# irfanfadhullah/unet_zoo

Hardware: AMD Instinct MI355X
Metric: images/sec (fwd+bwd) at B=16 3x256x256, 1/2/4/8 MI355X (higher is better)
Workload: dtype bf16; 1 GPU; unet train step (zero_grad+fwd+BCE+bwd+clip+AdamW), B=16/GPU 3x256x256, random-init weights; global_batch=16, parallelism=dp1

## Files before the change

unet_zoo_amd/csrc/uz_common.h:

```cpp
#pragma once
#include <hip/hip_runtime.h>
#include <stdarg.h>
#include <stdint.h>
#include <stdio.h>
#include "../../include/unetzoo_hip.h"

typedef __bf16 bf16_t;
typedef __attribute__((ext_vector_type(16))) float f32x16;
typedef __attribute__((ext_vector_type(4))) float f32x4;
typedef __attribute__((ext_vector_type(8))) __bf16 bf16x8;
typedef __attribute__((ext_vector_type(4))) __bf16 bf16x4;

#include <hip/hip_ext.h>
bool uz_prof_take(hipEvent_t* e0, hipEvent_t* e1);
#undef hipLaunchKernelGGL
#define hipLaunchKernelGGL(kern, grid, block, shm, stream, ...)                                              \
  do {                                                                                                       \
    hipEvent_t uz_e0_, uz_e1_;                                                                               \
    if (uz_prof_take(&uz_e0_, &uz_e1_))                                                                      \
      hipExtLaunchKernelGGL(kern, dim3(grid), dim3(block), (shm), (stream), uz_e0_, uz_e1_, 0, __VA_ARGS__);   \
    else                                                                                                     \
      kern<<<dim3(grid), dim3(block), (shm), (stream)>>>(__VA_ARGS__);                                       \
  } while (0)

// ... 109 lines not shown
  const char* e = getenv("UZ_TUNE");
  return e ? atoi(e) : 0;
}
static inline const char* uz_ablate_env(const char* name) { return getenv(name); }
#else
static inline int uz_tune_flags() { return 0; }
static inline const char* uz_ablate_env(const char*) { return nullptr; }
#endif

struct UzDirectPlan {
  int tw, bn, bres, th_n, tw_n, ntiles, tiles_n, grid_m;
  int ppcfg;
  int ksplit, cps;
};
int uz_direct_plan(const uz_conv_desc* d, UzDirectPlan* p);
struct UzBnRed {
  const void* y;
  int ldy;
  const float *scale, *shift, *mean, *invstd;
};
struct UzXf {
  const float *scale, *shift;
};
struct UzBnAct {
  const float *scale, *shift;
  int relu;
};
int uz_direct_launch(const uz_conv_desc* d, const UzDirectPlan& p, const void* x, const void* w,
                     const float* bias, void* y, float* stats, hipStream_t s, const UzBnRed* br = nullptr,
                     float* part = nullptr,
                     const UzXf* xf = nullptr, const UzBnAct* ba = nullptr);

enum { UZ_PP_512 = 0,
       UZ_PP_512X64 = 1,
       UZ_PP_256 = 2,
       UZ_PP_256W16 = 3,
       UZ_PP_128W16 = 4 };
struct UzPpPlan {
  int cfg, bn, th_n, tw_n, ntiles, tiles_n, grid_m;
  int ksplit, cps;
};
int uz_pp_plan(const uz_conv_desc* d, UzPpPlan* p);
int uz_pp_launch(const uz_conv_desc* d, const UzPpPlan& p, const void* x, const void* w, const float* bias, void* y,
                 float* stats, hipStream_t s, const UzBnRed* br = nullptr, float* part = nullptr, const UzXf* xf = nullptr,
                 const UzBnAct* ba = nullptr);
int uz_pp_xf_channels(const UzPpPlan& p);

struct UzWgrad2Plan {
  int big, one_tap, gather, kw, kr, tiles_i, tiles_j, kg, units, upb, split, nslabs, H, W;
  int wide9;
  int v9, bi;
};
int uz_wgrad9_plan(const uz_wgrad_desc* d, UzWgrad2Plan* p);
int uz_wgrad9_launch(const uz_wgrad_desc* d, const UzWgrad2Plan& p, const void* L, const void* R, float* slab, hipStream_t s,
                     const UzXf* xf = nullptr);
const char* uz_wgrad9_name(const UzWgrad2Plan& p);
int uz_wgrad_g4_plan(const uz_wgrad_desc* d, UzWgrad2Plan* p);
int uz_wgrad_g4_launch(const uz_wgrad_desc* d, const UzWgrad2Plan& p, const void* L, const void* R, float* slab, hipStream_t s);
int uz_wgrad3x3_plan(const uz_wgrad_desc* d, UzWgrad2Plan* p, int batch = 1);
int uz_wgrad3x3_launch(const uz_wgrad_desc* d, const UzWgrad2Plan& p, const void* L, const void* R,
                       float* slab, hipStream_t s, int batch = 1, long long lb_bytes = 0, long long rb_bytes = 0,
                       long long slab_stride = 0,
                       int batch2 = 1, long long lb2_bytes = 0, long long rb2_bytes = 0,
                       const UzXf* xf = nullptr);

struct UzWgradMultiItem {
  const uz_wgrad_desc* d;
  UzWgrad2Plan p;
  const void *L, *R;
  float* slab;
};
int uz_wgrad3x3_multi_max();
int uz_wgrad3x3_multi_launch(const UzWgradMultiItem* items, int n, hipStream_t s);

struct UzGemmPlan {
  int bn, bm, nst, tiles_m, tiles_n, grid_m;
  int ksplit, cps;
};
int uz_gemm_dma_plan(const uz_conv_desc* d, UzGemmPlan* p);
long long uz_gemm_dma_workspace_bytes(const uz_conv_desc* d);
int uz_gemm_dma_launch(const uz_conv_desc* d, const UzGemmPlan& p, const void* x, const void* w,
                       const float* bias, void* y, float* stats, hipStream_t s, const void* res = nullptr,
                       int ldres = 0, const UzBnRed* br = nullptr, float* part = nullptr);
```

unet_zoo_amd/csrc/uz_igemm.hip:

```cpp
#include "uz_common.h"
#include <string.h>

namespace {

struct IgemmArgs {
  const void* x;
  const void* w;
  void* y;
  const float* bias;
  float* stats;
  int M, H, W, Hin, Win, Cin, ldx, Nout, ldy, K, ntaps, mode, dil, store, Co, tiles_m, Hout, Wout;
  float* part;
  int tpg;
  const float* act_scale;
  const float* act_shift;
  int act_relu;
};

template <typename T> struct Mma;
template <> struct Mma<bf16_t> {
  static __device__ __forceinline__ void run(const Vec16<bf16_t>& a, const Vec16<bf16_t>& b,
                                             f32x16& c) {
    c = __builtin_amdgcn_mfma_f32_32x32x16_bf16(*reinterpret_cast<const bf16x8*>(&a),
                                                *reinterpret_cast<const bf16x8*>(&b), c, 0, 0, 0);
// ... 373 lines not shown
    UZ_REQUIRE(d->dil >= 1, "uz_conv_igemm: dil=%d", d->dil);
  } else if (d->taps_mode == UZ_TAPS_CONV_S2) {
    UzGemmPlan gs2_;
    UZ_REQUIRE(d->ntaps == 9 && d->store_mode == UZ_STORE_PLAIN && d->H == (d->Hin + 1) / 2 && d->W == (d->Win + 1) / 2,
               "uz_conv_igemm: stride-2 taps need ntaps=9, a plain store and H = ceil(Hin/2), W = ceil(Win/2)");
    UZ_REQUIRE(uz_gemm_dma_plan(d, &gs2_), "uz_conv_igemm: stride-2 taps need the LDS-DMA GEMM (channel multiples, tensor < 2 GiB)");
  } else {
    UZ_REQUIRE(d->taps_mode == UZ_TAPS_GATHER2X2 && d->ntaps == 4,
               "uz_conv_igemm: gather2x2 needs ntaps=4");
    UZ_REQUIRE((d->Hin == 2 * d->H || d->Hin == 2 * d->H + 1) && (d->Win == 2 * d->W || d->Win == 2 * d->W + 1),
               "uz_conv_igemm: gather2x2 needs Hin in {2H, 2H+1}, Win in {2W, 2W+1}");
  }
  if (d->store_mode == UZ_STORE_SHUFFLE2X2) {
    UZ_REQUIRE(d->Co > 0 && d->Nout == 4 * d->Co, "uz_conv_igemm: shuffle store needs Nout=4*Co");
    UZ_REQUIRE((d->Hout == 0 || d->Hout == 2 * d->H || d->Hout == 2 * d->H + 1) &&
                   (d->Wout == 0 || d->Wout == 2 * d->W || d->Wout == 2 * d->W + 1),
               "uz_conv_igemm: shuffle store destination must be 2H..2H+1 x 2W..2W+1");
    UZ_REQUIRE(d->ldy >= d->Co, "uz_conv_igemm: bad ldy");
  } else {
    UZ_REQUIRE(d->store_mode == UZ_STORE_PLAIN, "uz_conv_igemm: bad store_mode");
    UZ_REQUIRE(d->ldy >= d->Nout, "uz_conv_igemm: bad ldy=%d (Nout=%d)", d->ldy, d->Nout);
  }
  const long long M = (long long)d->N * d->H * d->W;
  UZ_REQUIRE(M * (long long)(d->ldx > d->ldy ? d->ldx : d->ldy) < (1LL << 40) && M < (1LL << 31),
             "uz_conv_igemm: tensor too large");
  UZ_REQUIRE((long long)d->N * d->Hin * d->Win < (1LL << 31), "uz_conv_igemm: input too large");
  p->bn = d->Nout <= 64 ? 64 : 128;
  p->tiles_m = uz_cdiv(M, 128);
  p->tiles_n = uz_cdiv(d->Nout, p->bn);
  int cap = (2 * UZ_NUM_CU) / p->tiles_n;
  if (cap < 1) cap = 1;
  p->grid_m = p->tiles_m < cap ? p->tiles_m : cap;
  p->split = 1;
  const int vec_ = d->dtype == UZ_BF16 ? 8 : 4;
  if (d->taps_mode == UZ_TAPS_CONV && d->ntaps == 9 && d->store_mode == UZ_STORE_PLAIN &&
      p->tiles_m * p->tiles_n <= UZ_NUM_CU / 2 && d->Nout % vec_ == 0 && d->ldy % vec_ == 0 &&
      !(uz_tune_flags() & 8)) {
    p->split = 9;
    reduce_geometry(M, d->Nout, vec_, p);
  }
  return UZ_OK;
}

template <typename T>
int launch(const uz_conv_desc* d, const Plan& p, const IgemmArgs& a, hipStream_t s) {
  dim3 grid(p.grid_m, p.tiles_n, a.part != nullptr ? p.split : 1), block(256);
  if (a.act_scale != nullptr) {
    if (p.bn == 64) hipLaunchKernelGGL((igemm_kernel<T, 128, 64, 2, 2, true>), grid, block, 0, s, a);
    else hipLaunchKernelGGL((igemm_kernel<T, 128, 128, 2, 2, true>), grid, block, 0, s, a);
    UZ_LAUNCH_CHECK("uz_conv_igemm_bnact");
    return UZ_OK;
  }
  if (p.bn == 64) {
    hipLaunchKernelGGL((igemm_kernel<T, 128, 64, 2, 2>), grid, block, 0, s, a);
  } else {
    hipLaunchKernelGGL((igemm_kernel<T, 128, 128, 2, 2>), grid, block, 0, s, a);
  }
  UZ_LAUNCH_CHECK("uz_conv_igemm");
  if (a.part != nullptr) {
    constexpr int VEC = ElemTraits<T>::VEC;
    const size_t shm = (size_t)256 * 2 * VEC * sizeof(float);
    hipLaunchKernelGGL((igemm_split_reduce_kernel<T>), dim3(p.rgx, p.rgy), dim3(p.rbx, p.rby), shm, s,
                       static_cast<const float*>(a.part), p.split, a.M, a.Nout, a.bias, static_cast<T*>(a.y), a.ldy, a.stats,
                       static_cast<const T*>(nullptr), 0);
    UZ_LAUNCH_CHECK("uz_conv_igemm(split reduce)");
  }
  return UZ_OK;
}

bool generic_path(const uz_conv_desc* d) {
  UzDirectPlan dp;
  UzGemmPlan gp;
  return !uz_direct_plan(d, &dp) && !uz_gemm_dma_plan(d, &gp);
}

}

extern "C" int uz_conv_igemm_grid_m(const uz_conv_desc* d) {
  Plan p;
  const int rc = make_plan(d, &p);
  if (rc != UZ_OK) return rc;
  UzDirectPlan dp;
  if (uz_direct_plan(d, &dp)) return dp.grid_m;
  UzGemmPlan gp;
  if (uz_gemm_dma_plan(d, &gp)) return gp.grid_m;
  return p.grid_m;
}

extern "C" int uz_conv_igemm_kernel_name(const uz_conv_desc* d, int with_workspace, char* buf, int cap) {
  Plan p;
  const int rc = make_plan(d, &p);
  if (rc != UZ_OK) return rc;
  UZ_REQUIRE(buf != nullptr && cap > 0, "uz_conv_igemm_kernel_name: no buffer");
  const char* dt = d->dtype == UZ_BF16 ? "bf16" : "f32";
  char name[96];
  UzDirectPlan dp;
  UzGemmPlan gp;
  if (uz_direct_plan(d, &dp)) {
    const char* up = d->taps_mode == UZ_TAPS_CONV_UP2 ? "_up2" : "";
    static const char* const ppn[8] = {"pp512", "pp512x64", "pp256", "pp256w16", "pp128w16", "?", "?", "?"};
    if (dp.bres == 3) snprintf(name, sizeof(name), "conv3x3_%s_%s%s%s", ppn[dp.ppcfg & 7], dt, up, (dp.ksplit > 1 && with_workspace) ? "_splitk" : "");
    else if (dp.bres == 2) snprintf(name, sizeof(name), "conv3x3_res64_%s%s", dt, up);
    else snprintf(name, sizeof(name), "conv3x3_direct_%s_bn%d%s%s", dt, dp.bn, dp.bres == 1 ? "_resident" : "", up);
  } else if (uz_gemm_dma_plan(d, &gp)) {
    snprintf(name, sizeof(name), "gemm_dma_%s", dt);
  } else {
    snprintf(name, sizeof(name), "igemm_%s_128x%d%s", dt, p.bn, (p.split > 1 && with_workspace) ? "_tapsplit" : "");
  }
  const int len = (int)strlen(name);
  snprintf(buf, (size_t)cap, "%s", name);
  return len;
}

extern "C" long long uz_conv_igemm_workspace_bytes(const uz_conv_desc* d) {
  Plan p;
  const int rc = make_plan(d, &p);
  if (rc != UZ_OK) return rc;
  {
    UzDirectPlan dp;
    if (uz_direct_plan(d, &dp) && dp.bres == 3 && dp.ksplit > 1)
      return (long long)dp.ksplit * d->N * d->H * d->W * d->Nout * (long long)sizeof(float);
  }
  {
    UzDirectPlan dp;
    const long long gb = uz_direct_plan(d, &dp) ? 0 : uz_gemm_dma_workspace_bytes(d);
    if (gb > 0) return gb;
  }
  if (p.split <= 1 || !generic_path(d)) return 0;
  return (long long)p.split * d->N * d->H * d->W * d->Nout * (long long)sizeof(float);
}

extern "C" int uz_conv_igemm_ws_grid_m(const uz_conv_desc* d) {
  Plan p;
  const int rc = make_plan(d, &p);
  if (rc != UZ_OK) return rc;
  {
    UzDirectPlan dp;
    if (uz_direct_plan(d, &dp) && dp.bres == 3 && dp.ksplit > 1) {
      Plan rp;
      reduce_geometry((long long)d->N * d->H * d->W, d->Nout, 8, &rp);
      return rp.rgx;
    }
  }
  {
    UzDirectPlan dp;
    if (!uz_direct_plan(d, &dp) && uz_gemm_dma_workspace_bytes(d) > 0) {
      Plan rp;
      reduce_geometry((long long)d->N * d->H * d->W, d->Nout, 8, &rp);
      return rp.rgx;
    }
  }
  if (p.split > 1 && generic_path(d)) return p.rgx;
  return uz_conv_igemm_grid_m(d);
}

extern "C" int uz_conv_igemm(const uz_conv_desc* d, const void* x, const void* w_packed,
                             const float* bias, void* y, float* stats_partial, void* stream) {
  return uz_conv_igemm_ws(d, x, w_packed, bias, y, stats_partial, nullptr, stream);
}

static int gemm_split_k(const uz_conv_desc* d, const UzGemmPlan& gp, const void* x, const void* w_packed, const float* bias,
                        const void* res, int ldres, void* y, void* workspace, hipStream_t s, float* stats = nullptr) {
  const int r1 = uz_gemm_dma_launch(d, gp, x, w_packed, nullptr, y, nullptr, s, nullptr, 0, nullptr, static_cast<float*>(workspace));
  if (r1 != UZ_OK) return r1;
  Plan rp;
  const long long M = (long long)d->N * d->H * d->W;
  reduce_geometry(M, d->Nout, 8, &rp);
  const size_t shm = (size_t)256 * 2 * 8 * sizeof(float);
  hipLaunchKernelGGL((igemm_split_reduce_kernel<bf16_t>), dim3(rp.rgx, rp.rgy), dim3(rp.rbx, rp.rby), shm, s,
                     static_cast<const float*>(workspace), gp.ksplit, (int)M, d->Nout, bias, static_cast<bf16_t*>(y), d->ldy,
                     stats, static_cast<const bf16_t*>(res), ldres);
  UZ_LAUNCH_CHECK("uz_conv_igemm(split-K GEMM reduce)");
  return UZ_OK;
}

extern "C" int uz_conv_igemm_res(const uz_conv_desc* d, const void* x, const void* w_packed, const float* bias,
                                 const void* res, int ldres, void* y, void* stream) {
  return uz_conv_igemm_res_ws(d, x, w_packed, bias, res, ldres, y, nullptr, stream);
}

extern "C" int uz_conv_igemm_res_ws(const uz_conv_desc* d, const void* x, const void* w_packed, const float* bias,
                                    const void* res, int ldres, void* y, void* workspace, void* stream) {
  Plan p;
  const int rc = make_plan(d, &p);
  if (rc != UZ_OK) return rc;
  UZ_REQUIRE(x && w_packed && y && res, "uz_conv_igemm_res: null pointer");
  UZ_REQUIRE(((uintptr_t)x & 15) == 0 && ((uintptr_t)w_packed & 15) == 0 && ((uintptr_t)y & 15) == 0 &&
                 ((uintptr_t)res & 15) == 0, "uz_conv_igemm_res: x / w / y / res must be 16-byte aligned");
  const int vec = d->dtype == UZ_BF16 ? 8 : 4;
  UZ_REQUIRE(ldres >= d->Nout && ldres % vec == 0, "uz_conv_igemm_res: bad ldres %d", ldres);
  UzDirectPlan dp;
  UzGemmPlan gp;
  if (d->store_mode != UZ_STORE_PLAIN || uz_direct_plan(d, &dp) || !uz_gemm_dma_plan(d, &gp)) {
    uz_set_error("uz_conv_igemm_res: only problems of the LDS-DMA GEMM with a plain store take a residual");
    return UZ_ENOTIMPL;
  }
  if (gp.ksplit > 1 && workspace != nullptr)
    return gemm_split_k(d, gp, x, w_packed, bias, res, ldres, y, workspace, static_cast<hipStream_t>(stream));
  return uz_gemm_dma_launch(d, gp, x, w_packed, bias, y, nullptr, static_cast<hipStream_t>(stream), res, ldres);
}

extern "C" int uz_conv_igemm_xf_supported(const uz_conv_desc* d) {
  UzDirectPlan dp;
  if (d == nullptr || d->dtype != UZ_BF16) return 0;
  if (!uz_direct_plan(d, &dp) || dp.bres != 3 || dp.ksplit > 1) return 0;
  UzPpPlan pp = {dp.ppcfg, dp.bn, dp.th_n, dp.tw_n, dp.ntiles, dp.tiles_n, dp.grid_m, dp.ksplit, dp.cps};
  return d->Cin <= uz_pp_xf_channels(pp) ? 1 : 0;
}

extern "C" int uz_conv_igemm_xf(const uz_conv_desc* d, const void* x, const float* in_scale, const float* in_shift,
                                const void* w_packed, const float* bias, void* y, float* stats_partial, void* stream) {
  Plan p;
  const int rc = make_plan(d, &p);
  if (rc != UZ_OK) return rc;
  UZ_REQUIRE(x && w_packed && y && in_scale && in_shift, "uz_conv_igemm_xf: null pointer");
  UZ_REQUIRE(((uintptr_t)x & 15) == 0 && ((uintptr_t)w_packed & 15) == 0 && ((uintptr_t)y & 15) == 0,
             "uz_conv_igemm_xf: x / w / y must be 16-byte aligned");
  if (!uz_conv_igemm_xf_supported(d)) {
    uz_set_error("uz_conv_igemm_xf: only bf16 3x3 problems of the ping-pong configurations whose LDS image leaves room for "
                 "the channel table (ask uz_conv_igemm_xf_supported)");
    return UZ_ENOTIMPL;
  }
  UzDirectPlan dp;
  UZ_REQUIRE(uz_direct_plan(d, &dp), "uz_conv_igemm_xf: no plan");
  const UzXf xf = {in_scale, in_shift};
  return uz_direct_launch(d, dp, x, w_packed, bias, y, stats_partial, static_cast<hipStream_t>(stream), nullptr, nullptr, &xf);
}

extern "C" int uz_conv_igemm_bnred_supported(const uz_conv_desc* d) {
  UzDirectPlan dp;
  UzGemmPlan gp;
  if (d == nullptr || d->dtype != UZ_BF16) return 0;
  if (uz_direct_plan(d, &dp)) return dp.bres != 2 ? 1 : 0;
  return (d->store_mode == UZ_STORE_PLAIN && uz_gemm_dma_plan(d, &gp)) ? 1 : 0;
}

extern "C" int uz_conv_igemm_bnred(const uz_conv_desc* d, const void* x, const void* w_packed, void* y,
                                   const void* bn_y, int ld_bny, const float* scale, const float* shift,
                                   const float* mean, const float* invstd, float* partial, void* stream) {
  Plan p;
  const int rc = make_plan(d, &p);
  if (rc != UZ_OK) return rc;
  UZ_REQUIRE(x && w_packed && y && bn_y && scale && shift && mean && invstd && partial,
             "uz_conv_igemm_bnred: null pointer");
  UZ_REQUIRE(((uintptr_t)x & 15) == 0 && ((uintptr_t)w_packed & 15) == 0 && ((uintptr_t)y & 15) == 0 &&
                 ((uintptr_t)bn_y & 15) == 0, "uz_conv_igemm_bnred: x / w / y / bn_y must be 16-byte aligned");
  UZ_REQUIRE(ld_bny >= d->Nout && ld_bny % 8 == 0, "uz_conv_igemm_bnred: bad ld_bny %d", ld_bny);
  UzDirectPlan dp;
  UzGemmPlan gp;
  if (!uz_conv_igemm_bnred_supported(d)) {
    uz_set_error("uz_conv_igemm_bnred: only bf16 problems of the direct 3x3 kernels with the LDS-staged epilogue and of "
                 "the LDS-DMA GEMM with a plain store (ask uz_conv_igemm_bnred_supported)");
    return UZ_ENOTIMPL;
  }
  const UzBnRed br = {bn_y, ld_bny, scale, shift, mean, invstd};
  if (uz_direct_plan(d, &dp))
    return uz_direct_launch(d, dp, x, w_packed, nullptr, y, partial, static_cast<hipStream_t>(stream), &br);
  UZ_REQUIRE(uz_gemm_dma_plan(d, &gp), "uz_conv_igemm_bnred: no plan");
  return uz_gemm_dma_launch(d, gp, x, w_packed, nullptr, y, partial, static_cast<hipStream_t>(stream), nullptr, 0, &br);
}

extern "C" int uz_conv_igemm_ws(const uz_conv_desc* d, const void* x, const void* w_packed,
                                const float* bias, void* y, float* stats_partial, void* workspace,
                                void* stream) {
  Plan p;
  const int rc = make_plan(d, &p);
  if (rc != UZ_OK) return rc;
  UZ_REQUIRE(x && w_packed && y, "uz_conv_igemm: null pointer");
  UZ_REQUIRE(((uintptr_t)x & 15) == 0 && ((uintptr_t)w_packed & 15) == 0 && ((uintptr_t)y & 15) == 0,
             "uz_conv_igemm: x / w / y must be 16-byte aligned");
  UzDirectPlan dp;
  if (uz_direct_plan(d, &dp)) {
    if (dp.bres == 3 && dp.ksplit > 1 && workspace != nullptr) {
      hipStream_t s = static_cast<hipStream_t>(stream);
      const int r1 = uz_direct_launch(d, dp, x, w_packed, nullptr, y, nullptr, s, nullptr, static_cast<float*>(workspace));
      if (r1 != UZ_OK) return r1;
      Plan rp;
      const long long M = (long long)d->N * d->H * d->W;
      reduce_geometry(M, d->Nout, 8, &rp);
      const size_t shm = (size_t)256 * 2 * 8 * sizeof(float);
      hipLaunchKernelGGL((igemm_split_reduce_kernel<bf16_t>), dim3(rp.rgx, rp.rgy), dim3(rp.rbx, rp.rby), shm, s,
                         static_cast<const float*>(workspace), dp.ksplit, (int)M, d->Nout, bias, static_cast<bf16_t*>(y), d->ldy,
                         stats_partial, static_cast<const bf16_t*>(nullptr), 0);
      UZ_LAUNCH_CHECK("uz_conv_igemm(split-K reduce)");
      return UZ_OK;
    }
    return uz_direct_launch(d, dp, x, w_packed, bias, y, stats_partial, static_cast<hipStream_t>(stream));
  }
  UzGemmPlan gp;
  if (uz_gemm_dma_plan(d, &gp)) {
    if (gp.ksplit > 1 && workspace != nullptr)
      return gemm_split_k(d, gp, x, w_packed, bias, nullptr, 0, y, workspace, static_cast<hipStream_t>(stream), stats_partial);
    return uz_gemm_dma_launch(d, gp, x, w_packed, bias, y, stats_partial, static_cast<hipStream_t>(stream));
  }
  IgemmArgs a;
  a.x = x;
  a.w = w_packed;
  a.y = y;
  a.bias = bias;
  a.stats = stats_partial;
  a.M = d->N * d->H * d->W;
  a.H = d->H;
  a.W = d->W;
  a.Hin = d->Hin;
  a.Win = d->Win;
  a.Cin = d->Cin;
  a.ldx = d->ldx;
  a.Nout = d->Nout;
  a.ldy = d->ldy;
  a.K = d->ntaps * d->Cin;
  a.ntaps = d->ntaps;
  a.mode = d->taps_mode;
  a.dil = d->dil;
  a.store = d->store_mode;
  a.Co = d->Co;
  a.Hout = d->Hout ? d->Hout : 2 * d->H;
  a.Wout = d->Wout ? d->Wout : 2 * d->W;
  a.tiles_m = p.tiles_m;
  a.part = (p.split > 1 && workspace != nullptr) ? static_cast<float*>(workspace) : nullptr;
  a.tpg = (d->ntaps + p.split - 1) / p.split;
  a.act_scale = nullptr;
  a.act_shift = nullptr;
  a.act_relu = 0;
  hipStream_t s = static_cast<hipStream_t>(stream);
  return d->dtype == UZ_BF16 ? launch<bf16_t>(d, p, a, s) : launch<float>(d, p, a, s);
}

extern "C" int uz_conv_igemm_bnact_supported(const uz_conv_desc* d) {
  Plan p;
  if (d == nullptr || make_plan(d, &p) != UZ_OK) return 0;
  if (d->store_mode != UZ_STORE_PLAIN || !(d->taps_mode == UZ_TAPS_CONV || d->taps_mode == UZ_TAPS_CONV_UP2)) return 0;
  UzDirectPlan dp;
  UzGemmPlan gp;
  if (uz_direct_plan(d, &dp)) {
    if (dp.bres == 2) return 0;
    if (dp.bres == 3 && dp.ksplit > 1) return 0;
    return 1;
  }
  if (uz_gemm_dma_plan(d, &gp)) return 0;
  return p.split > 1 ? 0 : 1;
}

extern "C" int uz_conv_igemm_bnact(const uz_conv_desc* d, const void* x, const void* w_packed, const float* bias,
                                   const float* out_scale, const float* out_shift, int relu, void* y, void* stream) {
  Plan p;
  const int rc = make_plan(d, &p);
  if (rc != UZ_OK) return rc;
  UZ_REQUIRE(x && w_packed && y && out_scale && out_shift, "uz_conv_igemm_bnact: null pointer");
  UZ_REQUIRE(((uintptr_t)x & 15) == 0 && ((uintptr_t)w_packed & 15) == 0 && ((uintptr_t)y & 15) == 0 &&
                 ((uintptr_t)out_scale & 15) == 0 && ((uintptr_t)out_shift & 15) == 0,
             "uz_conv_igemm_bnact: x / w / y / out_scale / out_shift must be 16-byte aligned");
  if (!uz_conv_igemm_bnact_supported(d)) {
    uz_set_error("uz_conv_igemm_bnact: only plain-store 3x3 / 1x1 problems of the direct kernels with a workgroup-wide "
                 "epilogue and of the generic kernel, without a split plan (ask uz_conv_igemm_bnact_supported)");
    return UZ_ENOTIMPL;
  }
  hipStream_t s = static_cast<hipStream_t>(stream);
  const UzBnAct ba = {out_scale, out_shift, relu ? 1 : 0};
  UzDirectPlan dp;
  if (uz_direct_plan(d, &dp)) return uz_direct_launch(d, dp, x, w_packed, bias, y, nullptr, s, nullptr, nullptr, nullptr, &ba);
  IgemmArgs a;
  a.x = x;
  a.w = w_packed;
  a.y = y;
  a.bias = bias;
  a.stats = nullptr;
  a.M = d->N * d->H * d->W;
  a.H = d->H;
  a.W = d->W;
  a.Hin = d->Hin;
  a.Win = d->Win;
// ... 21 lines not shown
```

unet_zoo_amd/ops.py:

```python
from __future__ import annotations

import ctypes
import math
from ctypes import byref
from typing import List, Optional, Sequence

import torch

from . import _lib as L


class Act:

    __slots__ = ("buf", "off", "C", "N", "H", "W", "grads", "parts", "rparts", "needs_grad", "colsums", "bn_src",
                 "bn_partials", "lazy", "_taken")

    def __init__(self, buf: torch.Tensor, off: int, C: int, N: int, H: int, W: int, needs_grad: bool = True):
        assert buf.dim() == 2 and buf.is_contiguous() and buf.shape[0] == N * H * W
        assert 0 <= off and off + C <= buf.shape[1]
        self.buf, self.off, self.C, self.N, self.H, self.W = buf, off, C, N, H, W
        self.grads: List["Act"] = []
        self.parts: Optional[Sequence["Act"]] = None
        self.rparts: Optional[Sequence[tuple]] = None
        self.needs_grad = needs_grad
# ... 221 lines not shown

def conv_first_wgrad(x: torch.Tensor, dy: Act, out: Optional[torch.Tensor] = None) -> torch.Tensor:
    L.require_cuda(x, dy.buf)
    N, C, H, W = x.shape
    Cout = dy.C
    lib = L.load()
    ws_bytes = L.check_count(lib.uz_conv3x3_first_wgrad_workspace_bytes(N, H, W, Cout), "uz_conv3x3_first_wgrad_workspace_bytes")
    ws = torch.empty(ws_bytes // 4, dtype=torch.float32, device=x.device)
    if out is None:
        out = torch.empty((Cout, C, 3, 3), dtype=torch.float32, device=x.device)
    assert out.numel() == Cout * C * 9 and out.is_contiguous() and out.dtype == torch.float32
    with _Timed("wgrad_first_bf16", 2.0 * N * H * W * 9 * C * Cout, 4.0 * x.numel() + 2.0 * dy.P * Cout):
        L.check(lib.uz_conv3x3_first_wgrad(L.dtype_code(dy.dtype), x.data_ptr(), N, C, H, W, dy.ptr(), dy.ld, Cout,
                                           out.data_ptr(), ws.data_ptr(), L.stream_ptr()), "uz_conv3x3_first_wgrad")
    return out


def conv_first_wgrad_bn(x: torch.Tensor, g: Act, y: Act, vec: torch.Tensor, sums: torch.Tensor,
                        out: Optional[torch.Tensor] = None) -> torch.Tensor:
    L.require_cuda(x, g.buf, y.buf)
    N, C, H, W = x.shape
    Cout = g.C
    assert (y.N, y.H, y.W, y.C) == (g.N, g.H, g.W, g.C) == (N, H, W, Cout) and g.dtype == y.dtype == torch.bfloat16
    assert sums.dtype == torch.float64 and sums.shape == (2, Cout) and sums.is_contiguous()
    lib = L.load()
    ws_bytes = L.check_count(lib.uz_conv3x3_first_wgrad_workspace_bytes(N, H, W, Cout), "uz_conv3x3_first_wgrad_workspace_bytes")
    ws = torch.empty(ws_bytes // 4, dtype=torch.float32, device=x.device)
    if out is None:
        out = torch.empty((Cout, C, 3, 3), dtype=torch.float32, device=x.device)
    assert out.numel() == Cout * C * 9 and out.is_contiguous() and out.dtype == torch.float32
    with _Timed("wgrad_first_bf16", 2.0 * N * H * W * 9 * C * Cout, 4.0 * x.numel() + 4.0 * g.P * Cout):
        L.check(lib.uz_conv3x3_first_wgrad_bn(L.dtype_code(g.dtype), x.data_ptr(), N, C, H, W, g.ptr(), g.ld, y.ptr(), y.ld,
                                              vec[0].data_ptr(), vec[1].data_ptr(), vec[2].data_ptr(), vec[3].data_ptr(),
                                              sums.data_ptr(), float(y.P), Cout, out.data_ptr(), ws.data_ptr(), L.stream_ptr()),
                "uz_conv3x3_first_wgrad_bn")
    return out


def conv_kernel_name(d, with_workspace: bool = False) -> str:
    buf = ctypes.create_string_buffer(96)
    L.check_count(L.load().uz_conv_igemm_kernel_name(byref(d), 1 if with_workspace else 0, buf, 96),
                  "uz_conv_igemm_kernel_name")
    return buf.value.decode()


def _conv_desc(x: Act, nout: int, ldy: int, ntaps: int, taps_mode: int, dil: int = 1, store_mode: int = L.STORE_PLAIN,
               co: int = 0, Hd: int = 0, Wd: int = 0):
    if taps_mode == L.TAPS_CONV:
        H, W = x.H, x.W
    elif taps_mode == L.TAPS_CONV_UP2:
        H, W = 2 * x.H, 2 * x.W
    elif taps_mode == L.TAPS_CONV_S2:
        H, W = (x.H + 1) // 2, (x.W + 1) // 2
    else:
        H, W = x.H // 2, x.W // 2
    return L.ConvDesc(L.dtype_code(x.dtype), x.N, H, W, x.H, x.W, x.C, x.ld, nout, ldy, ntaps, taps_mode, dil, store_mode, co,
                      Hd, Wd)


def _wgrad_desc(Lt: Act, Rt: Act, ntaps: int, taps_mode: int = L.TAPS_CONV, dil: int = 1):
    return L.WgradDesc(L.dtype_code(Lt.dtype), Lt.N, Lt.H, Lt.W, Rt.H, Rt.W, Lt.C, Lt.ld, Rt.C, Rt.ld, ntaps, taps_mode, dil)


def conv_igemm(x: Act, w_packed: torch.Tensor, bias: Optional[torch.Tensor], y: Act, *,
               ntaps: int, dil: int = 1, taps_mode: int = L.TAPS_CONV,
               store_mode: int = L.STORE_PLAIN, nout: Optional[int] = None, co: int = 0,
               want_stats: bool = False, res: Optional[Act] = None,
               bnred: Optional[tuple] = None, xform: Optional[tuple] = None) -> Optional[torch.Tensor]:
    L.require_cuda(x.buf, w_packed, y.buf)
    lib = L.load()
    shuffle = store_mode == L.STORE_SHUFFLE2X2
    d = _conv_desc(x, nout if nout is not None else y.C, y.ld, ntaps, taps_mode, dil, store_mode, co,
                   y.H if shuffle else 0, y.W if shuffle else 0)
    assert w_packed.dtype == x.dtype and y.dtype == x.dtype
    assert w_packed.shape == (d.Nout, ntaps * x.C), (tuple(w_packed.shape), d.Nout, ntaps, x.C)
    stats = None
    if want_stats:
        gm = L.check_count(lib.uz_conv_igemm_ws_grid_m(byref(d)), "uz_conv_igemm_ws_grid_m")
        stats = torch.empty((gm, 2, d.Nout), dtype=torch.float32, device=x.buf.device)
    wsb = L.check_count(lib.uz_conv_igemm_workspace_bytes(byref(d)), "uz_conv_igemm_workspace_bytes")
    ws = torch.empty(wsb // 4, dtype=torch.float32, device=x.buf.device) if wsb > 0 else None
    M, K, es = d.N * d.H * d.W, ntaps * x.C, x.buf.element_size()
    kname = conv_kernel_name(d, ws is not None)
    if xform is not None:
        assert bnred is None and res is None
        with _Timed(kname + "_xf", 2.0 * M * d.Nout * K, es * (x.P * x.C + M * d.Nout + d.Nout * K)):
            L.check(lib.uz_conv_igemm_xf(byref(d), x.raw_ptr(), xform[0].data_ptr(), xform[1].data_ptr(), w_packed.data_ptr(),
                                         _p(bias), y.ptr(), _p(stats), L.stream_ptr()), "uz_conv_igemm_xf")
        return stats
    if bnred is not None:
        assert bias is None and res is None and not want_stats
        bn_y, vec4 = bnred
        if not lib.uz_conv_igemm_bnred_supported(byref(d)) or (bn_y.P, bn_y.C) != (y.P, y.C):
            bnred = None
        else:
            gm = L.check_count(lib.uz_conv_igemm_grid_m(byref(d)), "uz_conv_igemm_grid_m")
            part = torch.empty((gm, 2, d.Nout), dtype=torch.float32, device=x.buf.device)
            with _Timed(kname + "_bnred", 2.0 * M * d.Nout * K, es * (x.P * x.C + 2 * M * d.Nout + d.Nout * K)):
                L.check(lib.uz_conv_igemm_bnred(byref(d), x.ptr(), w_packed.data_ptr(), y.ptr(), bn_y.ptr(), bn_y.ld,
                                                vec4[0].data_ptr(), vec4[1].data_ptr(), vec4[2].data_ptr(),
                                                vec4[3].data_ptr(), part.data_ptr(), L.stream_ptr()),
                        "uz_conv_igemm_bnred")
            return part
    if res is not None:
        assert (res.P, res.C) == (y.P, y.C) and res.dtype == y.dtype and not want_stats
        if kname.startswith("gemm_dma") and store_mode == L.STORE_PLAIN:
            with _Timed(kname, 2.0 * M * d.Nout * K, es * (x.P * x.C + 2 * M * d.Nout + d.Nout * K)):
                L.check(lib.uz_conv_igemm_res_ws(byref(d), x.ptr(), w_packed.data_ptr(), _p(bias), res.ptr(), res.ld, y.ptr(),
                                                 _p(ws), L.stream_ptr()), "uz_conv_igemm_res_ws")
            return None
    with _Timed(kname, 2.0 * M * d.Nout * K,
                        es * (x.P * x.C + M * d.Nout + d.Nout * K)):
        L.check(lib.uz_conv_igemm_ws(byref(d), x.ptr(), w_packed.data_ptr(), _p(bias), y.ptr(), _p(stats),
                                     _p(ws), L.stream_ptr()), "uz_conv_igemm_ws")
    if res is not None:
        add_acts(y, res, y)
    return stats


def conv_bnact_supported(x: Act, nout: int, ldy: int, *, ntaps: int, dil: int = 1, taps_mode: int = L.TAPS_CONV) -> bool:
    if taps_mode not in (L.TAPS_CONV, L.TAPS_CONV_UP2):
        return False
    d = _conv_desc(x, nout, ldy, ntaps, taps_mode, dil)
    return bool(L.load().uz_conv_igemm_bnact_supported(byref(d)))


def conv_igemm_bnact(x: Act, w_packed: torch.Tensor, bias: Optional[torch.Tensor], scale: torch.Tensor, shift: torch.Tensor,
                     relu: bool, y: Act, *, ntaps: int, dil: int = 1, taps_mode: int = L.TAPS_CONV) -> None:
    L.require_cuda(x.buf, w_packed, y.buf, scale, shift)
    d = _conv_desc(x, y.C, y.ld, ntaps, taps_mode, dil)
    assert w_packed.dtype == x.dtype and y.dtype == x.dtype and (y.N, y.H, y.W) == (d.N, d.H, d.W)
    assert w_packed.shape == (d.Nout, ntaps * x.C), (tuple(w_packed.shape), d.Nout, ntaps, x.C)
    assert scale.dtype == shift.dtype == torch.float32 and scale.numel() == shift.numel() == d.Nout
    assert scale.is_contiguous() and shift.is_contiguous()
    M, K, es = d.N * d.H * d.W, ntaps * x.C, x.buf.element_size()
    with _Timed(conv_kernel_name(d) + "_bnact", 2.0 * M * d.Nout * K, es * (x.P * x.C + M * d.Nout + d.Nout * K)):
        L.check(L.load().uz_conv_igemm_bnact(byref(d), x.ptr(), w_packed.data_ptr(), _p(bias), scale.data_ptr(),
                                             shift.data_ptr(), 1 if relu else 0, y.ptr(), L.stream_ptr()), "uz_conv_igemm_bnact")


def conv_first_fwd_bnact(x: torch.Tensor, w: torch.Tensor, bias: Optional[torch.Tensor], scale: torch.Tensor,
                         shift: torch.Tensor, relu: bool, y: Act) -> None:
    L.require_cuda(x, w, y.buf, scale, shift)
    assert x.dtype == torch.float32 and x.is_contiguous() and w.dtype == torch.float32 and w.is_contiguous()
    N, C, H, W = x.shape
    Cout = w.shape[0]
    assert (y.N, y.H, y.W, y.C) == (N, H, W, Cout) and tuple(w.shape) == (Cout, C, 3, 3)
    assert scale.dtype == shift.dtype == torch.float32 and scale.numel() == shift.numel() == Cout
    assert scale.is_contiguous() and shift.is_contiguous()
    with _Timed("conv3x3_first_bf16_bnact", 2.0 * N * H * W * 9 * C * Cout, 4.0 * x.numel() + 2.0 * y.P * Cout):
        L.check(L.load().uz_conv3x3_first_fwd_bnact(L.dtype_code(y.dtype), x.data_ptr(), N, C, H, W, w.data_ptr(), _p(bias), Cout,
                                                    scale.data_ptr(), shift.data_ptr(), 1 if relu else 0, y.ptr(), y.ld,
                                                    L.stream_ptr()), "uz_conv3x3_first_fwd_bnact")


def conv_xform_supported(x: Act, nout: int, ldy: int, *, upsample: bool = False) -> bool:
    d = _conv_desc(x, nout, ldy, 9, L.TAPS_CONV_UP2 if upsample else L.TAPS_CONV)
    return bool(L.load().uz_conv_igemm_xf_supported(byref(d)))


def wgrad_kernel_name(d) -> str:
    buf = ctypes.create_string_buffer(96)
    L.check_count(L.load().uz_wgrad_kernel_name(byref(d), buf, 96), "uz_wgrad_kernel_name")
    return buf.value.decode()


def wgrad_xform_supported(Lt: Act, Rt: Act, ntaps: int, *, taps_mode: int = L.TAPS_CONV, dil: int = 1) -> bool:
    return bool(L.load().uz_wgrad_xf_supported(byref(_wgrad_desc(Lt, Rt, ntaps, taps_mode, dil))))


def wgrad_xform_shapes_supported(N: int, H: int, W: int, Ci: int, ldl: int, Cj: int, ldr: int, dtype: torch.dtype) -> bool:
    def shape(C, ld):
        return Act(torch.empty((N * H * W, ld), dtype=dtype, device="meta"), 0, C, N, H, W)
    return wgrad_xform_supported(shape(Ci, ldl), shape(Cj, ldr), 9)


def wgrad(Lt: Act, Rt: Act, out_shape, *, ntaps: int, dil: int = 1,
          taps_mode: int = L.TAPS_CONV, out: Optional[torch.Tensor] = None, xform: Optional[tuple] = None) -> torch.Tensor:
    L.require_cuda(Lt.buf, Rt.buf)
    lib = L.load()
    d = _wgrad_desc(Lt, Rt, ntaps, taps_mode, dil)
    ws_bytes = L.check_count(lib.uz_wgrad_workspace_bytes(byref(d)), "uz_wgrad_workspace_bytes")
    ws = torch.empty(ws_bytes // 4, dtype=torch.float32, device=Lt.buf.device)
    if out is None:
        out = torch.empty(out_shape, dtype=torch.float32, device=Lt.buf.device)
    assert out.numel() == Lt.C * Rt.C * ntaps and out.is_contiguous() and out.dtype == torch.float32
    def run(phase):
        if xform is not None:
            L.check(lib.uz_wgrad_xf(byref(d), Lt.ptr(), Rt.raw_ptr(), xform[0].data_ptr(), xform[1].data_ptr(), out.data_ptr(),
# ... 1263 lines not shown
```

Before: 2675 images/sec.

## Add dedicated MFMA kernel for 2x2 transposed conv forward and gather dgrad

```diff
diff --git a/unet_zoo_amd/csrc/uz_common.h b/unet_zoo_amd/csrc/uz_common.h
--- a/unet_zoo_amd/csrc/uz_common.h
+++ b/unet_zoo_amd/csrc/uz_common.h
@@ -215,3 +215,10 @@
 int uz_gemm_dma_launch(const uz_conv_desc* d, const UzGemmPlan& p, const void* x, const void* w,
                        const float* bias, void* y, float* stats, hipStream_t s, const void* res = nullptr,
                        int ldres = 0, const UzBnRed* br = nullptr, float* part = nullptr);
+
+struct UzConvtPlan {
+  int dgrad, level, tiles, grid_m;
+};
+int uz_convt2x2_plan(const uz_conv_desc* d, UzConvtPlan* p);
+int uz_convt2x2_launch(const uz_conv_desc* d, const UzConvtPlan& p, const void* x, const void* w, const float* bias,
+                       void* y, hipStream_t s, const UzBnRed* br = nullptr, float* part = nullptr);
diff --git a/unet_zoo_amd/csrc/uz_convt2x2.hip b/unet_zoo_amd/csrc/uz_convt2x2.hip
--- /dev/null
+++ b/unet_zoo_amd/csrc/uz_convt2x2.hip
@@ -0,0 +1,314 @@
+#include "uz_common.h"
+
+namespace {
+
+struct CtArgs {
+  const bf16_t* x;
+  const bf16_t* w;
+  bf16_t* y;
+  const float* bias;
+  const bf16_t* bn_y;
+  const float *bn_scale, *bn_shift, *bn_mean, *bn_invstd;
+  float* part;
+  int ldx, ldy, ld_bny, H, W, Co, tiles;
+};
+
+enum { CT_FWD = 0, CT_DGRAD = 1, CT_DGRAD_BNRED = 2 };
+
+template <int KS, int NB, int NC, bool STREAM, bool PREF, int MODE>
+__global__ __launch_bounds__(512, 1) void convt2x2_kernel(const CtArgs a) {
+  constexpr int K = KS * 16, KB = K * 2;
+  constexpr int CH = NB * 32, NOUT = NC * CH;
+  constexpr int CHUNK = CH * KB;
+  constexpr int WBYTES = STREAM ? 2 * CHUNK : NC * CHUNK;
+  constexpr int RS = CH * 2 + 16, STRIP = 32 * RS;
+  constexpr int U = CH / 8;
+  constexpr int NPASS = U / 2, RPP = 64 / U;
+  constexpr int FP = CH * (K / 8) / 512;
+  constexpr int VOFF = WBYTES + 8 * STRIP;
+  constexpr int NVEC = MODE == CT_DGRAD_BNRED ? 2 : 1;
+  constexpr bool BNRED = MODE == CT_DGRAD_BNRED;
+  constexpr int UNR = PREF ? NC : 1;
+  static_assert(!STREAM || NC % 2 == 0, "a streamed chunk's buffer is its parity");
+  static_assert(FP >= 1 && FP * 512 == CH * (K / 8), "chunk fill");
+  static_assert(MODE == CT_FWD || KS % 4 == 0, "four taps");
+  static_assert(!BNRED || (2 * NOUT <= 512 && NB == 2), "BatchNorm-backward sums");
+  constexpr int TOFF = VOFF + NVEC * NOUT * 4;
+  __shared__ __attribute__((aligned(16))) char smem[TOFF + (BNRED ? 8 * 2 * 4 * NOUT * 4 : 0)];
+
+  const int tid = threadIdx.x, lane = tid & 63;
+  const int wave = __builtin_amdgcn_readfirstlane(tid >> 6);
+  const int l31 = lane & 31, lh = lane >> 5;
+  const int HW = a.H * a.W;
+  const int Wf = 2 * a.W;
+  auto prow = [&](int sr) { return BNRED ? 32 * (sr >> 2) + 4 * wave + (sr & 3) : wave * 32 + sr; };
+
+  auto wload = [&](int c, Vec16<bf16_t> (&r)[FP]) {
+#pragma unroll
+    for (int p = 0; p < FP; ++p) {
+      const unsigned u = p * 512 + tid;
+      r[p] = *reinterpret_cast<const Vec16<bf16_t>*>(reinterpret_cast<const char*>(a.w + (size_t)c * CH * K) + u * 16);
+    }
+  };
+  auto wstore = [&](char* buf, const Vec16<bf16_t> (&r)[FP]) {
+#pragma unroll
+    for (int p = 0; p < FP; ++p) {
+      const int u = p * 512 + tid, row = u / (K / 8), kc = u % (K / 8);
+      *reinterpret_cast<Vec16<bf16_t>*>(buf + (kc >> 3) * (CH * 128) + row * 128 + (((kc & 7) ^ ((row >> 1) & 7)) << 4)) = r[p];
+    }
+  };
+  auto aload = [&](int t, Vec16<bf16_t> (&r)[KS]) {
+    const int m = t * 256 + prow(l31);
+    if constexpr (MODE == CT_FWD) {
+      const bf16_t* p = a.x + (size_t)m * a.ldx + lh * 8;
+#pragma unroll
+      for (int kk = 0; kk < KS; ++kk) r[kk] = ld16(p + kk * 16);
+    } else {
+      const int img = m / HW, rem = m - img * HW;
+      const int h = rem / a.W, w = rem - h * a.W;
+      const int fp = (img * 2 * a.H + 2 * h) * Wf + 2 * w;
+#pragma unroll
+      for (int tap = 0; tap < 4; ++tap) {
+        const bf16_t* p = a.x + (size_t)(fp + (tap >> 1) * Wf + (tap & 1)) * a.ldx + lh * 8;
+#pragma unroll
+        for (int kk = 0; kk < KS / 4; ++kk) r[tap * (KS / 4) + kk] = ld16(p + kk * 16);
+      }
+    }
+  };
+
+  {
+    float* sv = reinterpret_cast<float*>(smem + VOFF);
+    for (int i = tid; i < NOUT; i += 512) {
+      if constexpr (BNRED) {
+        sv[i] = a.bn_scale[i];
+        sv[NOUT + i] = a.bn_shift[i];
+        for (int k = 0; k < 64; ++k) reinterpret_cast<float*>(smem + TOFF)[k * NOUT + i] = 0.f;
+      } else {
+        sv[i] = a.bias != nullptr ? a.bias[i] : 0.f;
+      }
+    }
+    Vec16<bf16_t> w0[FP];
+    for (int c = 0; c < (STREAM ? 1 : NC); ++c) {
+      wload(c, w0);
+      wstore(smem + c * CHUNK, w0);
+    }
+  }
+  Vec16<bf16_t> cur[KS], nxt[PREF ? KS : 1];
+  if constexpr (PREF) aload(blockIdx.x, cur);
+  __syncthreads();
+
+  int qoff[4];
+#pragma unroll
+  for (int q = 0; q < 4; ++q) qoff[q] = l31 * 128 + (((2 * q + lh) ^ ((l31 >> 1) & 7)) << 4);
+  char* strip = smem + WBYTES + wave * STRIP;
+  const int cc = lane % U, r0 = lane / U;
+  auto srow = [&](int k) { return BNRED ? 16 * (r0 >> 2) + 4 * k + (r0 & 3) : r0 + k * RPP; };
+  float* tot = reinterpret_cast<float*>(smem + TOFF) + wave * 8 * NOUT + (r0 & 3) * NOUT;
+
+  for (int tile = blockIdx.x; tile < a.tiles; tile += gridDim.x) {
+    if constexpr (PREF) {
+      const int nt = tile + (int)gridDim.x;
+      aload(nt < a.tiles ? nt : tile, nxt);
+    } else {
+      aload(tile, cur);
+    }
+    unsigned yoff[NPASS], boff[BNRED ? NPASS : 1];
+#pragma unroll
+    for (int k = 0; k < NPASS; ++k) {
+      const int m = tile * 256 + prow(srow(k));
+      if constexpr (MODE == CT_FWD) {
+        const int img = m / HW, rem = m - img * HW;
+        const int h = rem / a.W, w = rem - h * a.W;
+        yoff[k] = (unsigned)((img * 2 * a.H + 2 * h) * Wf + 2 * w) * (unsigned)(a.ldy * 2) + cc * 16;
+      } else {
+        yoff[k] = (unsigned)m * (unsigned)(a.ldy * 2) + cc * 16;
+        if constexpr (BNRED) boff[k] = (unsigned)m * (unsigned)(a.ld_bny * 2) + cc * 16;
+      }
+    }
+
+#pragma unroll UNR
+    for (int c = 0; c < NC; ++c) {
+      const char* wb = smem + (STREAM ? (c & 1) : c) * CHUNK;
+      Vec16<bf16_t> wr[STREAM ? FP : 1];
+      if constexpr (STREAM) wload(c + 1 < NC ? c + 1 : 0, wr);
+      const int n0 = c * CH;
+
+      f32x16 acc[NB];
+#pragma unroll
+      for (int j = 0; j < NB; ++j)
+#pragma unroll
+        for (int r = 0; r < 16; ++r) acc[j][r] = 0.f;
+#pragma unroll
+      for (int kk = 0; kk < KS; ++kk) {
+#pragma unroll
+        for (int j = 0; j < NB; ++j) {
+          const bf16x8 wf = *reinterpret_cast<const bf16x8*>(wb + (kk >> 2) * (CH * 128) + j * 4096 + qoff[kk & 3]);
+          acc[j] = __builtin_amdgcn_mfma_f32_32x32x16_bf16(wf, *reinterpret_cast<const bf16x8*>(&cur[kk]), acc[j], 0, 0, 0);
+        }
+      }
+
+      if constexpr (STREAM) wstore(smem + ((c + 1) & 1) * CHUNK, wr);
+
+      Vec16<bf16_t> yb[BNRED ? NPASS : 1];
+      if constexpr (BNRED) {
+#pragma unroll
+        for (int k = 0; k < NPASS; ++k)
+          yb[k] = *reinterpret_cast<const Vec16<bf16_t>*>(reinterpret_cast<const char*>(a.bn_y + n0) + boff[k]);
+      }
+      const float* sv = reinterpret_cast<const float*>(smem + VOFF);
+#pragma unroll
+      for (int j = 0; j < NB; ++j)
+#pragma unroll
+        for (int q = 0; q < 4; ++q) {
+          bf16x4 pk;
+          if constexpr (BNRED) {
+#pragma unroll
+            for (int e = 0; e < 4; ++e) pk[e] = (bf16_t)acc[j][4 * q + e];
+          } else {
+            const f32x4 bq = *reinterpret_cast<const f32x4*>(sv + n0 + j * 32 + 8 * q + 4 * lh);
+#pragma unroll
+            for (int e = 0; e < 4; ++e) pk[e] = (bf16_t)(acc[j][4 * q + e] + bq[e]);
+          }
+          *reinterpret_cast<bf16x4*>(strip + l31 * RS + (j * 32 + 8 * q + 4 * lh) * 2) = pk;
+        }
+      Vec16<bf16_t> vb[NPASS];
+#pragma unroll
+      for (int k = 0; k < NPASS; ++k) vb[k] = *reinterpret_cast<const Vec16<bf16_t>*>(strip + srow(k) * RS + cc * 16);
+      if constexpr (MODE == CT_FWD) {
+        const int ab = n0 / a.Co, co = n0 - ab * a.Co;
+        char* yc = reinterpret_cast<char*>(a.y + (size_t)((ab >> 1) * Wf + (ab & 1)) * a.ldy + co);
+#pragma unroll
+        for (int k = 0; k < NPASS; ++k) *reinterpret_cast<Vec16<bf16_t>*>(yc + yoff[k]) = vb[k];
+      } else {
+        char* yc = reinterpret_cast<char*>(a.y + n0);
+#pragma unroll
+        for (int k = 0; k < NPASS; ++k) *reinterpret_cast<Vec16<bf16_t>*>(yc + yoff[k]) = vb[k];
+      }
+      if constexpr (BNRED) {
+        const bool upper = (r0 >> 2) != 0;
+#pragma unroll
+        for (int eh = 0; eh < 8; eh += 4) {
+          const f32x4 bsc = *reinterpret_cast<const f32x4*>(sv + n0 + cc * 8 + eh);
+          const f32x4 bsh = *reinterpret_cast<const f32x4*>(sv + NOUT + n0 + cc * 8 + eh);
+          f32x4* t1 = reinterpret_cast<f32x4*>(tot + n0 + cc * 8 + eh);
+          f32x4* t2 = reinterpret_cast<f32x4*>(tot + 4 * NOUT + n0 + cc * 8 + eh);
+          f32x4 s1 = *t1, s2 = *t2;
+#pragma unroll
+          for (int half = 0; half < 2; ++half) {
+            if (half == 1) {
+#pragma unroll
+              for (int e = 0; e < 4; ++e) {
+                s1[e] = __shfl_xor(s1[e], 32);
+                s2[e] = __shfl_xor(s2[e], 32);
+              }
+            }
+#pragma unroll
+            for (int k = 0; k < NPASS; ++k)
+#pragma unroll
+              for (int e = 0; e < 4; ++e) {
+                const float yv = (float)yb[k].v[eh + e];
+                const float dz = fmaf(yv, bsc[e], bsh[e]) > 0.f ? (float)vb[k].v[eh + e] : 0.f;
+                s1[e] += dz;
+                s2[e] += dz * yv;
+              }
+          }
+          if (upper) {
+            *t1 = s1;
+            *t2 = s2;
+          }
+        }
+      }
+      if constexpr (STREAM) {
+        asm volatile("s_waitcnt lgkmcnt(0)" ::: "memory");
+        __builtin_amdgcn_s_barrier();
+        asm volatile("" ::: "memory");
+      }
+    }
+    if constexpr (PREF) {
+#pragma unroll
+      for (int kk = 0; kk < KS; ++kk) cur[kk] = nxt[kk];
+    }
+  }
+
+  if constexpr (BNRED) {
+    __syncthreads();
+    const float* red = reinterpret_cast<const float*>(smem + TOFF);
+    if (tid < 2 * NOUT) {
+      const int which = tid / NOUT, ch = tid - which * NOUT;
+      float t = 0.f;
+      for (int r = 0; r < 32; ++r) t += red[(((r >> 2) * 2 + which) * 4 + (r & 3)) * NOUT + ch];
+      if (which == 1) {
+        float t0 = 0.f;
+        for (int r = 0; r < 32; ++r) t0 += red[((r >> 2) * 2 * 4 + (r & 3)) * NOUT + ch];
+        t = a.bn_invstd[ch] * (t - a.bn_mean[ch] * t0);
+      }
+      a.part[((size_t)blockIdx.x * 2 + which) * NOUT + ch] = t;
+    }
+  }
+}
+
+}
+
+int uz_convt2x2_plan(const uz_conv_desc* d, UzConvtPlan* p) {
+  if (d->dtype != UZ_BF16 || d->dil != 1) return 0;
+  const long long M = (long long)d->N * d->H * d->W;
+  if (M <= 0 || M % 256 != 0 || 4 * M >= (1LL << 31)) return 0;
+  if (d->ldx % 8 != 0 || d->ldy % 8 != 0 || d->ldx < d->Cin) return 0;
+  if (4 * M * d->ldy * 2 >= (1LL << 32)) return 0;
+  if (d->store_mode == UZ_STORE_SHUFFLE2X2 && d->taps_mode == UZ_TAPS_CONV && d->ntaps == 1) {
+    if (d->Hin != d->H || d->Win != d->W) return 0;
+    if ((d->Hout != 0 && d->Hout != 2 * d->H) || (d->Wout != 0 && d->Wout != 2 * d->W)) return 0;
+    if (d->Co % 64 != 0 || d->Nout != 4 * d->Co || d->ldy < d->Co) return 0;
+    if (d->Cin == 128 && d->Co == 64) p->level = 1;
+    else if (d->Cin == 256 && d->Co == 128) p->level = 2;
+    else return 0;
+    p->dgrad = 0;
+  } else if (d->store_mode == UZ_STORE_PLAIN && d->taps_mode == UZ_TAPS_GATHER2X2 && d->ntaps == 4) {
+    if (d->Hin != 2 * d->H || d->Win != 2 * d->W || d->ldy < d->Nout) return 0;
+    if (d->Cin == 64 && d->Nout == 128) p->level = 1;
+    else return 0;
+    p->dgrad = 1;
+  } else {
+    return 0;
+  }
+  p->tiles = (int)(M / 256);
+  p->grid_m = p->tiles < UZ_NUM_CU ? p->tiles : UZ_NUM_CU;
+  return 1;
+}
+
+int uz_convt2x2_launch(const uz_conv_desc* d, const UzConvtPlan& p, const void* x, const void* w, const float* bias,
+                       void* y, hipStream_t s, const UzBnRed* br, float* part) {
+  CtArgs a;
+  a.x = static_cast<const bf16_t*>(x);
+  a.w = static_cast<const bf16_t*>(w);
+  a.y = static_cast<bf16_t*>(y);
+  a.bias = bias;
+  a.bn_y = br ? static_cast<const bf16_t*>(br->y) : nullptr;
+  a.bn_scale = br ? br->scale : nullptr;
+  a.bn_shift = br ? br->shift : nullptr;
+  a.bn_mean = br ? br->mean : nullptr;
+  a.bn_invstd = br ? br->invstd : nullptr;
+  a.ld_bny = br ? br->ldy : 0;
+  a.part = part;
+  a.ldx = d->ldx;
+  a.ldy = d->ldy;
+  a.H = d->H;
+  a.W = d->W;
+  a.Co = d->Co;
+  a.tiles = p.tiles;
+  UZ_REQUIRE(br == nullptr || (p.dgrad && part != nullptr && bias == nullptr), "uz_conv_igemm_bnred(convt2x2): input gradient only");
+  UZ_REQUIRE(br == nullptr || (long long)d->N * d->H * d->W * br->ldy * 2 < (1LL << 32), "uz_conv_igemm_bnred(convt2x2): bn_y above 4 GiB");
+  dim3 grid(p.grid_m), block(512);
+  if (!p.dgrad) {
+    if (p.level == 1) hipLaunchKernelGGL((convt2x2_kernel<8, 2, 4, false, true, CT_FWD>), grid, block, 0, s, a);
+    else hipLaunchKernelGGL((convt2x2_kernel<16, 2, 8, true, false, CT_FWD>), grid, block, 0, s, a);
+    UZ_LAUNCH_CHECK("uz_conv_igemm(convt2x2_fwd)");
+  } else if (br == nullptr) {
+    hipLaunchKernelGGL((convt2x2_kernel<16, 2, 2, false, true, CT_DGRAD>), grid, block, 0, s, a);
+    UZ_LAUNCH_CHECK("uz_conv_igemm(convt2x2_dgrad)");
+  } else {
+    hipLaunchKernelGGL((convt2x2_kernel<16, 2, 2, false, true, CT_DGRAD_BNRED>), grid, block, 0, s, a);
+    UZ_LAUNCH_CHECK("uz_conv_igemm_bnred(convt2x2_dgrad)");
+  }
+  return UZ_OK;
+}
diff --git a/unet_zoo_amd/csrc/uz_igemm.hip b/unet_zoo_amd/csrc/uz_igemm.hip
--- a/unet_zoo_amd/csrc/uz_igemm.hip
+++ b/unet_zoo_amd/csrc/uz_igemm.hip
@@ -479,6 +479,8 @@
   if (rc != UZ_OK) return rc;
   UzDirectPlan dp;
   if (uz_direct_plan(d, &dp)) return dp.grid_m;
+  UzConvtPlan cp;
+  if (uz_convt2x2_plan(d, &cp)) return cp.grid_m;
   UzGemmPlan gp;
   if (uz_gemm_dma_plan(d, &gp)) return gp.grid_m;
   return p.grid_m;
@@ -493,12 +495,15 @@
   char name[96];
   UzDirectPlan dp;
   UzGemmPlan gp;
+  UzConvtPlan cp;
   if (uz_direct_plan(d, &dp)) {
     const char* up = d->taps_mode == UZ_TAPS_CONV_UP2 ? "_up2" : "";
     static const char* const ppn[8] = {"pp512", "pp512x64", "pp256", "pp256w16", "pp128w16", "?", "?", "?"};
     if (dp.bres == 3) snprintf(name, sizeof(name), "conv3x3_%s_%s%s%s", ppn[dp.ppcfg & 7], dt, up, (dp.ksplit > 1 && with_workspace) ? "_splitk" : "");
     else if (dp.bres == 2) snprintf(name, sizeof(name), "conv3x3_res64_%s%s", dt, up);
     else snprintf(name, sizeof(name), "conv3x3_direct_%s_bn%d%s%s", dt, dp.bn, dp.bres == 1 ? "_resident" : "", up);
+  } else if (uz_convt2x2_plan(d, &cp)) {
+    snprintf(name, sizeof(name), "convt2x2_%s_%s", cp.dgrad ? "dgrad" : "fwd", dt);
   } else if (uz_gemm_dma_plan(d, &gp)) {
     snprintf(name, sizeof(name), "gemm_dma_%s", dt);
   } else {
@@ -517,6 +522,10 @@
     UzDirectPlan dp;
     if (uz_direct_plan(d, &dp) && dp.bres == 3 && dp.ksplit > 1)
       return (long long)dp.ksplit * d->N * d->H * d->W * d->Nout * (long long)sizeof(float);
+  }
+  {
+    UzConvtPlan cp;
+    if (uz_convt2x2_plan(d, &cp)) return 0;
   }
   {
     UzDirectPlan dp;
@@ -548,6 +557,11 @@
     }
   }
   if (p.split > 1 && generic_path(d)) return p.rgx;
+  {
+    UzConvtPlan cp;
+    UzGemmPlan gp;
+    if (uz_convt2x2_plan(d, &cp) && uz_gemm_dma_plan(d, &gp)) return gp.grid_m;
+  }
   return uz_conv_igemm_grid_m(d);
 }
 
@@ -629,6 +643,8 @@
   UzGemmPlan gp;
   if (d == nullptr || d->dtype != UZ_BF16) return 0;
   if (uz_direct_plan(d, &dp)) return dp.bres != 2 ? 1 : 0;
+  UzConvtPlan cp;
+  if (uz_convt2x2_plan(d, &cp)) return cp.dgrad;
   return (d->store_mode == UZ_STORE_PLAIN && uz_gemm_dma_plan(d, &gp)) ? 1 : 0;
 }
 
@@ -653,6 +669,9 @@
   const UzBnRed br = {bn_y, ld_bny, scale, shift, mean, invstd};
   if (uz_direct_plan(d, &dp))
     return uz_direct_launch(d, dp, x, w_packed, nullptr, y, partial, static_cast<hipStream_t>(stream), &br);
+  UzConvtPlan cp;
+  if (uz_convt2x2_plan(d, &cp) && cp.dgrad)
+    return uz_convt2x2_launch(d, cp, x, w_packed, nullptr, y, static_cast<hipStream_t>(stream), &br, partial);
   UZ_REQUIRE(uz_gemm_dma_plan(d, &gp), "uz_conv_igemm_bnred: no plan");
   return uz_gemm_dma_launch(d, gp, x, w_packed, nullptr, y, partial, static_cast<hipStream_t>(stream), nullptr, 0, &br);
 }
@@ -684,6 +703,9 @@
     }
     return uz_direct_launch(d, dp, x, w_packed, bias, y, stats_partial, static_cast<hipStream_t>(stream));
   }
+  UzConvtPlan cp;
+  if (stats_partial == nullptr && uz_convt2x2_plan(d, &cp))
+    return uz_convt2x2_launch(d, cp, x, w_packed, bias, y, static_cast<hipStream_t>(stream));
   UzGemmPlan gp;
   if (uz_gemm_dma_plan(d, &gp)) {
     if (gp.ksplit > 1 && workspace != nullptr)
diff --git a/unet_zoo_amd/ops.py b/unet_zoo_amd/ops.py
--- a/unet_zoo_amd/ops.py
+++ b/unet_zoo_amd/ops.py
@@ -327,6 +327,8 @@
     ws = torch.empty(wsb // 4, dtype=torch.float32, device=x.buf.device) if wsb > 0 else None
     M, K, es = d.N * d.H * d.W, ntaps * x.C, x.buf.element_size()
     kname = conv_kernel_name(d, ws is not None)
+    if want_stats and kname.startswith("convt2x2"):
+        kname = "gemm_dma_bf16"
     if xform is not None:
         assert bnred is None and res is None
         with _Timed(kname + "_xf", 2.0 * M * d.Nout * K, es * (x.P * x.C + M * d.Nout + d.Nout * K)):
@@ -349,7 +351,9 @@
             return part
     if res is not None:
         assert (res.P, res.C) == (y.P, y.C) and res.dtype == y.dtype and not want_stats
-        if kname.startswith("gemm_dma") and store_mode == L.STORE_PLAIN:
+        if kname.startswith(("gemm_dma", "convt2x2")) and store_mode == L.STORE_PLAIN:
+            if kname.startswith("convt2x2"):
+                kname = "gemm_dma_bf16"
             with _Timed(kname, 2.0 * M * d.Nout * K, es * (x.P * x.C + 2 * M * d.Nout + d.Nout * K)):
                 L.check(lib.uz_conv_igemm_res_ws(byref(d), x.ptr(), w_packed.data_ptr(), _p(bias), res.ptr(), res.ld, y.ptr(),
                                                  _p(ws), L.stream_ptr()), "uz_conv_igemm_res_ws")
```

Result: no change. 2695 images/sec (median of 6 runs) (+0.7%).
